# EDAPINENUT/CBGBench

Measured on AMD Instinct MI355X. Metric: denoising graph-steps/s (pocket+ligand graphs x reverse-diffusion steps per second), higher is better.
Workload: dtype f32; 1 GPU; configs/denovo targetdiff sampling, BASELINE configs[1] job: 100 pockets x 10 samples = 1000 graphs per GPU, 3 resident batch(es) of <= 340; N_rec~U[350,650], N_lig~U[10,45], k=32, 9 layers; bench step = 1 reverse-diffusion step of the job at each of 5 time blocks; graphs_per_gpu=1000, nodes_per_gpu=521351, denoising_steps_per_bench_step=5, graph_steps_per_bench_step_per_gpu=5000, ranks_seen=1, launch=stream launches, streams=3, edge_workgroups=256, devices_by_uuid=1

## Files before the change

cbgbench_amd/csrc/api.hip:

```cpp
#include <hip/hip_runtime.h>

#include <cmath>
#include <cstdarg>
#include <cstdio>
#include <cstring>
#include <cstdlib>
#include <vector>

#include "../../include/cbgx.h"
#ifdef CBGX_XCHECK
#include "../../include/cbgx_xcheck.h"
#endif
#include "kernels.h"
#include "layout.h"
#include "workspace.h"

using namespace cbgx;

static thread_local char g_err[512] = "";

namespace cbgx {
int set_error(int code, const char* fmt, ...) {
    va_list ap;
    va_start(ap, fmt);
// ... 328 lines not shown
        HIP_TRY(launch_knn_reg(x, graph_ptr, n_graphs, n_nodes, w.nbr, w.deg, s, w.act.rows, w.act.count));
        HIP_TRY(launch_gate_mfma(packed, x, w.nbr, w.deg, n_nodes, w.e_w, s, w.act.rows, w.act.count));
    }
    NodeList src{nullptr, nullptr};
    if (g_edge_impl != 1) {
        HIP_TRY(launch_mark_seed(gen_flag, gen_flag, n_nodes, w.fa1, s));
        HIP_TRY(launch_mark_nbr(w.act.rows, w.act.count, n_nodes, w.nbr, w.deg, w.fa1, s));
        HIP_TRY(launch_build_active(w.fa1, n_nodes, w.A1.rows, w.A1.count, s));
        src = w.A1;
    }
    const float* xc = x;
    const NodeBufs& b = w.set[0];
    for (int l = 0; l < num_layers; ++l) {
        float* xn = (l == num_layers - 1) ? x_out : w.xbuf[l & 1];
        HIP_TRY(launch_attention(false, packed + GATE_SIZE + (size_t)l * ATT_SIZE, xc, h, w.nbr, w.deg, lig_flag, gen_flag,
                                 w.e_w, n_nodes, b.P, b.Qt, b.q, xn, nullptr, w.act.rows, w.act.count, src.rows, src.count, s));
        xc = xn;
    }
    return CBGX_OK;
}

size_t cbgx_workspace_bytes(int n_nodes, int n_graphs) {
    (void)n_graphs;
    return carve(nullptr, n_nodes).total;
}

int cbgx_knn_graph(const float* x, const int32_t* graph_ptr, int n_graphs, int n_nodes, int k, int32_t* nbr,
                   int32_t* deg, void* stream) {
    if (k != KNN) return fail(CBGX_E_INVALID, "knn_graph: only k=%d is supported (got %d)", KNN, k);
    if (n_nodes < 0 || n_graphs < 0) return fail(CBGX_E_INVALID, "knn_graph: negative size");
    if (n_nodes == 0) return CBGX_OK;
// ... 36 lines not shown
}

int cbgx_h2x_attention(const float* packed, int layer, const float* x, const float* h, const int32_t* nbr,
                       const int32_t* deg, const uint8_t* lig_flag, const uint8_t* gen_flag, const float* e_w,
                       int n_nodes, float* x_out, float* delta_x, void* workspace, size_t workspace_bytes,
                       void* stream) {
    if (n_nodes == 0) return CBGX_OK;
    if (!packed || !x || !h || !nbr || !deg || !lig_flag || !gen_flag || !e_w || !x_out || !workspace || layer < 0 ||
        n_nodes < 0)
        return fail(CBGX_E_INVALID, "h2x_attention: bad argument");
    Workspace w;
    if (int rc = carve_checked("h2x_attention", workspace, workspace_bytes, n_nodes, w)) return rc;
    const NodeBufs& b = w.set[0];
    HIP_TRY(launch_build_active(gen_flag, n_nodes, w.act.rows, w.act.count, (hipStream_t)stream));
    HIP_TRY(launch_attention(false, packed + h2x_off(layer), x, h, nbr, deg, lig_flag, gen_flag, e_w, n_nodes, b.P,
                             b.Qt, b.q, x_out, delta_x, w.act.rows, w.act.count, nullptr, nullptr, (hipStream_t)stream));
    return CBGX_OK;
}

int cbgx_node_stage(const float* packed, int layer, int x2h, const float* h, const uint8_t* lig_flag, int n_nodes,
                    const int32_t* rows, const int32_t* n_rows, int q_direct, float* P, float* q, float* Qt, void* stream) {
    if (n_nodes == 0) return CBGX_OK;
    if (!packed || !h || !lig_flag || !P || !q || !Qt || layer < 0 || n_nodes < 0 || (rows == nullptr) != (n_rows == nullptr))
        return fail(CBGX_E_INVALID, "node_stage: bad argument");
    HIP_TRY(launch_node_mfma(packed + (x2h ? x2h_off(layer) : h2x_off(layer)), h, lig_flag, n_nodes, P, q, Qt, rows, n_rows, nullptr,
                             nullptr, (hipStream_t)stream, true, nullptr, nullptr, q_direct != 0));
    return CBGX_OK;
}

static int classifier_head(const float* packed, int num_layers, int num_classes, const float* h, int n_nodes, float* hidden,
                           float* logits, NodeList rows, hipStream_t s) {
// ... 134 lines not shown
}

static hipError_t edge_x2h(const Forward& f, int l, const NodeBufs& b, const float* xc, const float* hc, float* hn) {
    const LayerPlan& p = f.plan[l];
    return launch_edge_x2h_dual(f.packed + x2h_off(l), xc, hc, b.P, b.Qt, b.q, f.w.nbr, f.w.deg, f.lig_flag, f.gen_flag, f.w.e_w,
                                f.n_nodes, hn, p.pp.rows, p.pp.count, p.gen.rows, p.gen.count, p.full_layer, f.s);
}
static hipError_t node_x2h(const Forward& f, int l, const NodeBufs& b, const float* h_in, hipStream_t on) {
    const LayerPlan& p = f.plan[l];
    return launch_node_mfma(f.packed + x2h_off(l), h_in, f.lig_flag, f.n_nodes, b.P, b.q, b.Qt, p.dst.rows, p.dst.count, p.src.rows,
                            p.src.count, on, true, p.gen.rows, p.gen.count, node_qdirect_enabled());
}
static hipError_t block_h2x(const Forward& f, int l, const NodeBufs& b, const float* xc, const float* hn, float* xn) {
    const Workspace& w = f.w;
    return launch_attention(false, f.packed + h2x_off(l), xc, hn, w.nbr, w.deg, f.lig_flag, f.gen_flag, w.e_w, f.n_nodes, b.P, b.Qt, b.q,
                            xn, nullptr, w.act.rows, w.act.count, w.A1.rows, w.A1.count, f.s);
}

static int forward_fused(const Forward& f) {
    const Workspace& w = f.w;
    hipStream_t s = f.s;
    auto add_x2h = [&](NodeStageJobs& jobs, int l) {
        const LayerPlan& p = f.plan[l];
        const NodeBufs& b = w.set[l & 1];
        add_node_stage_jobs(jobs, f.packed + x2h_off(l), b.P, b.q, b.Qt, p.dst.rows, p.dst.count, p.src.rows, p.src.count, p.fold_flag);
    };
    NodeStageJobs jobs;
    jobs.n = 0;
    add_x2h(jobs, 0);
    HIP_TRY(launch_node_stage_jobs(jobs, f.h, f.lig_flag, f.n_nodes, s));
    const float *xc = f.x, *hc = f.h;
    for (int l = 0; l < f.num_layers; ++l) {
        float *hn, *xn;
        HIP_TRY(begin_layer(f, l, hn, xn));
        HIP_TRY(edge_x2h(f, l, w.set[l & 1], xc, hc, hn));
        jobs.n = 0;
        add_node_stage_jobs(jobs, f.packed + h2x_off(l), w.set[2].P, w.set[2].q, w.set[2].Qt, w.act.rows, w.act.count, w.A1.rows,
                            w.A1.count);
        if (l + 1 < f.num_layers) add_x2h(jobs, l + 1);
        HIP_TRY(launch_node_stage_jobs(jobs, hn, f.lig_flag, f.n_nodes, s));
        HIP_TRY(launch_edge_mfma(false, f.packed + h2x_off(l), xc, hn, w.set[2].P, w.set[2].Qt, w.nbr, w.deg, f.lig_flag, f.gen_flag, w.e_w,
                                 f.n_nodes, xn, nullptr, w.act.rows, w.act.count, s));
        xc = xn;
        hc = hn;
    }
    return CBGX_OK;
}

static int forward_two_streams(const Forward& f, AuxStream* aux) {
    hipStream_t s = f.s;
    HIP_TRY(node_x2h(f, 0, f.w.set[0], f.h, s));
    const float *xc = f.x, *hc = f.h;
    for (int l = 0; l < f.num_layers; ++l) {
        float *hn, *xn;
        HIP_TRY(begin_layer(f, l, hn, xn));
        if (l > 0) HIP_TRY(hipStreamWaitEvent(s, aux->join, 0));
        HIP_TRY(edge_x2h(f, l, f.w.set[l & 1], xc, hc, hn));
// ... 276 lines not shown
```

cbgbench_amd/csrc/dispatch.hip:

```cpp
#include <hip/hip_runtime.h>
#include <stdint.h>

#include "kernels.h"
#include "layout.h"

namespace cbgx {

#ifdef CBGX_XCHECK
int g_edge_impl = 0;
#endif

#define CBGX_LAUNCH_CHECK()                            \
    do {                                               \
        hipError_t _e = hipGetLastError();             \
        if (_e != hipSuccess) return _e;               \
    } while (0)

hipError_t launch_knn(const float* x, const int32_t* graph_ptr, int n_graphs, int n_nodes, int32_t* nbr,
                      int32_t* deg, hipStream_t s) {
    if (n_nodes == 0) return hipSuccess;
#ifdef CBGX_XCHECK
    if (g_edge_impl == 1) return launch_knn_v1(x, graph_ptr, n_graphs, n_nodes, nbr, deg, s);
#endif
    return launch_knn_reg(x, graph_ptr, n_graphs, n_nodes, nbr, deg, s);
}

hipError_t launch_gate(const float* packed, const float* x, const int32_t* nbr, const int32_t* deg, int n_nodes,
                       float* e_w, hipStream_t s) {
    if (n_nodes == 0) return hipSuccess;
#ifdef CBGX_XCHECK
    if (g_edge_impl == 1) return launch_gate_v1(packed, x, nbr, deg, n_nodes, e_w, s);
#endif
    return launch_gate_mfma(packed, x, nbr, deg, n_nodes, e_w, s);
}

hipError_t launch_attention(bool x2h, const float* att, const float* x, const float* h, const int32_t* nbr,
                            const int32_t* deg, const uint8_t* lig, const uint8_t* gen, const float* e_w, int n_nodes,
                            float* P, float* Qt, float* qbuf, float* out, float* dx_out, const int* act, const int* act_count,
                            const int* src, const int* src_count, hipStream_t s) {
    if (n_nodes == 0) return hipSuccess;
#ifdef CBGX_XCHECK
    if (g_edge_impl == 1) return launch_attention_v1(x2h, att, x, h, nbr, deg, lig, gen, e_w, n_nodes, P, Qt, out, dx_out, s);
#endif
    hipError_t e0 = launch_node_mfma(att, h, lig, n_nodes, P, qbuf, Qt, act, act_count, src, src_count, s, x2h);
    if (e0 != hipSuccess) return e0;
    return launch_edge_mfma(x2h, att, x, h, P, Qt, nbr, deg, lig, gen, e_w, n_nodes, out, dx_out, act, act_count, s);
}

__global__ void pack_copy_kernel(const float* __restrict__ src, int src_ld, int src_off, int transpose,
                                 float* __restrict__ dst, int dst_ld, int rows, int cols) {
    int idx = blockIdx.x * blockDim.x + threadIdx.x;
    if (idx >= rows * cols) return;
    int i = idx / cols, j = idx % cols;
    dst[(size_t)i * dst_ld + j] = transpose ? src[(size_t)j * src_ld + i + src_off] : src[(size_t)i * src_ld + j + src_off];
}

__global__ void pack_copy_multi_kernel(PackBatch b) {
    const PackPiece& pc = b.p[blockIdx.y];
    const int total = pc.rows * pc.cols;
    for (int idx = blockIdx.x * blockDim.x + threadIdx.x; idx < total; idx += gridDim.x * blockDim.x) {
// ... 28 lines not shown
```

cbgbench_amd/csrc/edge_body.h:

```cpp
#pragma once
#include <hip/hip_runtime.h>
#include <stdint.h>

#include "edge_common.h"
#include "layout.h"

#ifndef CBGX_EDGE_MIN_WAVES
#define CBGX_EDGE_MIN_WAVES 2
#endif
#ifndef CBGX_EDGE_EARLY_HEADER
#define CBGX_EDGE_EARLY_HEADER 1
#endif
#ifndef CBGX_EDGE_EARLY_LOADS
#define CBGX_EDGE_EARLY_LOADS 1
#endif
#ifndef CBGX_EDGE_WAVE_MAJOR
#define CBGX_EDGE_WAVE_MAJOR 1
#endif

namespace cbgx {

constexpr int EDGE_MIN_WAVES = CBGX_EDGE_MIN_WAVES;
__host__ __device__ __forceinline__ int edge_active_waves(int n_items, int n_wg, int waves) {
    const int per_wg = (n_items + n_wg - 1) / (n_wg > 0 ? n_wg : 1);
// ... 114 lines not shown
        out0 = MFMA(fmaxf(ya.x, 0.f), bb.x, out0);
        out1 = MFMA(fmaxf(ya.y, 0.f), bb.y, out1);
        out0 = MFMA(fmaxf(yb.x, 0.f), bb.z, out0);
        out1 = MFMA(fmaxf(yb.y, 0.f), bb.w, out1);
    }
    return out0 + out1;
}

struct ItemGeom {
    int node, d, lig_i;
    float xi, yi, zi;
    int j0[2];
};
__device__ __forceinline__ int e1_id(int raw, int e, int d, int self) { return e < d ? raw : self; }

template <bool X2H, int WAVES, bool LISTED, bool PP, bool F16 = false>
__device__ __forceinline__ void edge_body(
    float* __restrict__ lds, float* __restrict__ lds_mu, const int wg, const int n_wg,
    const float* __restrict__ att, const float* __restrict__ x, const float* __restrict__ h,
    const float* __restrict__ P, const float* __restrict__ Qt, const int32_t* __restrict__ nbr,
    const int32_t* __restrict__ deg, const uint8_t* __restrict__ lig, const uint8_t* __restrict__ gen,
    const float* __restrict__ e_w, int n_nodes, float* __restrict__ out, float* __restrict__ dx_out,
    const int* __restrict__ act_arg, const int* __restrict__ act_count) {
    const int* __restrict__ act = LISTED ? act_arg : nullptr;
    static_assert(!PP || (X2H && LISTED), "the protein-only kernel is an x2h work-list kernel");
    static_assert(!F16 || X2H, "split-f16 scores and aggregation: x2h only");
    static_assert(PP_IMG_SIZE == IMG_SIZE_X2H, "both x2h images fill the same LDS array");
    constexpr int IMG = X2H ? (int)IMG_SIZE_X2H : (int)IMG_SIZE_H2X;
    auto copy_fixed_nodes = [&]() {
        if (!X2H && act) {
            for (int n = wg * (WAVES * 64) + threadIdx.x; n < n_nodes; n += n_wg * WAVES * 64) {
                unsigned gn = gen[n];
                float px = x[3 * n], py = x[3 * n + 1], pz = x[3 * n + 2];
                asm volatile("" : "+v"(gn), "+v"(px), "+v"(py), "+v"(pz));
                if (!gn) {
                    out[3 * n] = px; out[3 * n + 1] = py; out[3 * n + 2] = pz;
                    if (dx_out) { dx_out[3 * n] = 0.f; dx_out[3 * n + 1] = 0.f; dx_out[3 * n + 2] = 0.f; }
                }
            }
        }
    };
// ... 39 lines not shown
        const unsigned oc = vop(4 * c), oq = vop(16 * q);
        r0 = ldoi(nrow, oc); r1 = ldoi(nrow, oc + 64);
        nb0 = ldoi4(nrow, oq); nb1 = ldoi4(nrow, oq + 64);
    };
    {
        const floatx4* src = reinterpret_cast<const floatx4*>(att + (PP ? A_IMG_PP : A_IMG));
        floatx4* dst = reinterpret_cast<floatx4*>(lds);
        constexpr int NV = (IMG / 4 + WAVES * 64 - 1) / (WAVES * 64);
        if constexpr (WAVES >= 8) {
            floatx4 v[NV];
#pragma unroll
            for (int u = 0; u < NV; ++u) {
                const int t = threadIdx.x + u * (WAVES * 64);
                v[u] = src[t < IMG / 4 ? t : IMG / 4 - 1];
            }
            __builtin_amdgcn_sched_barrier(0);
            if (CBGX_EDGE_EARLY_HEADER && has_item) first_header();
            copy_fixed_nodes();
            __builtin_amdgcn_sched_barrier(0);
#pragma unroll
            for (int u = 0; u < NV; ++u) {
                const int t = threadIdx.x + u * (WAVES * 64);
                if (t < IMG / 4) dst[t] = v[u];
            }
        } else {
            if (CBGX_EDGE_EARLY_HEADER && has_item) first_header();
            copy_fixed_nodes();
            constexpr int NVC = 20;
#pragma unroll 1
            for (int u0 = 0; u0 < NV; u0 += NVC) {
                floatx4 v[NVC];
#pragma unroll
                for (int u = 0; u < NVC; ++u) {
                    const int t = threadIdx.x + (u0 + u) * (WAVES * 64);
                    v[u] = src[t < IMG / 4 ? t : IMG / 4 - 1];
                }
                __builtin_amdgcn_sched_barrier(0);
#pragma unroll
// ... 51 lines not shown
            dist0[hf] = edge_len(g.xi, g.yi, g.zi, ldo1(sbase(x), 12u * j), ldo1(sbase(x), 12u * j + 4), ldo1(sbase(x), 12u * j + 8));
        }
        const gptr pdp = sbase(P + (size_t)i * PROW);
        const unsigned o0 = (unsigned)g.j0[0] * (PROW * 4) + (2 * H + 4 * q) * 4, o1 = (unsigned)g.j0[1] * (PROW * 4) + (2 * H + 4 * q) * 4;
#pragma unroll
        for (int t = 0; t < 8; ++t) { pd[t] = ldo4(pdp, oq + 64 * t); ps0[t] = ldo4(sbase(P), o0 + 64 * t); }
#pragma unroll
        for (int t = 0; t < 8; ++t) ps1[t] = ldo4(sbase(P), o1 + 64 * t);
    }

    for (int k = i_begin; k < i_end; k += i_step) {
        const int i = __builtin_amdgcn_readfirstlane(g.node), d = g.d, lig_i = g.lig_i;
        const bool more = k + i_step < i_end;
        const int k_next = k + i_step;
        float4 q8a = {0.f, 0.f, 0.f, 0.f}, q8b = {0.f, 0.f, 0.f, 0.f};
        if (PP && CBGX_EDGE_EARLY_LOADS) {
            const gptr qp = sbase(Qt + (size_t)i * H);
            const unsigned oq8 = vop(32 * c);
            q8a = ldo4(qp, oq8); q8b = ldo4(qp, oq8 + 16);
        }
        floatx4 acc0[8], acc1[8];
#pragma unroll
        for (int t = 0; t < 8; ++t) {
            const floatx4 pds = f4(pd[t]) * sck.S;
            acc0[t] = f4(ps0[t]) * sck.S + pds; acc1[t] = f4(ps1[t]) * sck.S + pds;
        }
        __builtin_amdgcn_sched_barrier(0);
        ItemGeom ng;
        const int inext = __builtin_amdgcn_readfirstlane(more ? (act ? act[k_next] : k_next) : i);
        ng.node = inext;
        const int nd_raw = deg[inext];
        const int nlig_raw = PP ? 0 : ldob(sbase(lig), vop((unsigned)inext));
        const gptr xrow = sbase(x + 3 * (size_t)inext);
        const unsigned ozero = vop(0u);
        const float nx_raw = ldo1(xrow, ozero), ny_raw = ldo1(xrow, ozero + 4), nz_raw = ldo1(xrow, ozero + 8);
        const gptr nrow = sbase(nbr + (size_t)inext * KNN);
        const unsigned oc = vop(4 * c);
        const int nr0 = ldoi(nrow, oc), nr1 = ldoi(nrow, oc + 64);
        __builtin_amdgcn_sched_barrier(0);
        float4 qrow[8];
        if (PP && !CBGX_EDGE_EARLY_LOADS) {
            const gptr qp = sbase(Qt + (size_t)i * H);
            const unsigned oq8 = vop(32 * c);
            q8a = ldo4(qp, oq8); q8b = ldo4(qp, oq8 + 16);
        }
        if (!PP) {
            const gptr qp = sbase(Qt + (size_t)i * HEADS * H);
            const unsigned oqr = vop((c * H + 4 * q) * 4);
#pragma unroll
            for (int t = 0; t < 8; ++t) qrow[t] = ldo4(qp, oqr + 64 * t);
        }
        float4 sva[2][4], svb[2][4];
        float4 pa = {0.f, 0.f, 0.f, 0.f}, pb = {0.f, 0.f, 0.f, 0.f};
        if (X2H) {
            const int nbv[4] = {nb0.x, nb0.y, nb0.z, nb0.w};
#pragma unroll
            for (int r = 0; r < 4; ++r) {
                const unsigned o = (unsigned)e1_id(nbv[r], 4 * q + r, d, i) * (PROW * 4) + (3 * H + 4 * c) * 4;
                sva[0][r] = ldo4(sbase(P), o);
                svb[0][r] = ldo4(sbase(P), o + 256);
            }
// ... 9 lines not shown
            const float vm = c + 16 * hf < d ? RBF_UP : 0.f;
#pragma unroll
            for (int s = 0; s < 5; ++s) {
                const float u = dist0[hf] - lds_mu[4 * s + q];
                R[hf][s] = fast_exp(-0.5f * (u * u)) * vm;
            }
        }
        const unsigned long long b0 = __ballot(lg0[0]), b1 = __ballot(lg0[1]);
        const unsigned mask_lig = (unsigned)(b0 & 0xffffull) | ((unsigned)(b1 & 0xffffull) << 16);
        const unsigned mask_valid = d >= 32 ? 0xffffffffu : ((1u << d) - 1u);
        const bool has_lig = PP ? false : (mask_lig & mask_valid) != 0;
        const bool has_prot = PP ? true : ((~mask_lig) & mask_valid) != 0 || d == 0;

        floatx4 sc[2];
        float qun = 1.f;
        sc[0] = edge_major_half<true, PP, F16 ? 1 : 0>(acc0, lg0[0], 0, lds_fk, lds_dwt, lds_ln, R[0], has_prot, has_lig, lig_i, lane, q,
                                                       PP ? lds + PP_WFOLD + 4 * lane : nullptr, qrow, sck, q8a, q8b, khk_inv, &qun);
        __builtin_amdgcn_sched_barrier(0);
        int nlj[2];
        float nxj[2][3];
        {
            ng.d = __builtin_amdgcn_readfirstlane(nd_raw);
            ng.lig_i = __builtin_amdgcn_readfirstlane(nlig_raw);
            ng.xi = __uint_as_float(__builtin_amdgcn_readfirstlane(__float_as_uint(nx_raw)));
            ng.yi = __uint_as_float(__builtin_amdgcn_readfirstlane(__float_as_uint(ny_raw)));
            ng.zi = __uint_as_float(__builtin_amdgcn_readfirstlane(__float_as_uint(nz_raw)));
            ng.j0[0] = c < ng.d ? nr0 : inext;
            ng.j0[1] = c + 16 < ng.d ? nr1 : inext;
#pragma unroll
            for (int hf = 0; hf < 2; ++hf) {
                const int j = ng.j0[hf];
                nlj[hf] = PP ? 0 : ldob(sbase(lig), (unsigned)j);
// ... 320 lines not shown
```

cbgbench_amd/csrc/edge_mfma.hip:

```cpp
#include <hip/hip_runtime.h>
#include <stdint.h>

#include <stdlib.h>

#include <atomic>

#include "edge_common.h"
#include "kernels.h"
#include "layout.h"

namespace cbgx {


__constant__ float c_mu[G] = {0.f, 1.f, 1.25f, 1.5f, 1.75f, 2.f, 2.25f, 2.5f, 2.75f, 3.f,
                              3.5f, 4.f, 4.5f, 5.f, 5.5f, 6.f, 7.f, 8.f, 9.f, 10.f};

}

#include "edge_body.h"

namespace cbgx {

template <bool X2H, int WAVES, bool LISTED>
__global__ __launch_bounds__(WAVES * 64) void edge_mfma_kernel(
// ... 108 lines not shown
    const int idx = blockIdx.x * blockDim.x + threadIdx.x;
    if (idx >= H * H) return;
    if (!pb.x2h[blockIdx.y]) {
        if (idx >= HEADS * H) return;
        const int head = idx >> 7, m = idx & 127, t = m >> 4, q = (m >> 2) & 3, r = m & 3;
        pb.att[blockIdx.y][A_IMG + IMG_WBV + ((64 * t + 16 * q + head) << 2) + r] = pb.wv1[blockIdx.y][idx];
        return;
    }
    const int n = idx >> 7, m = idx & 127;
    const int chunk = 16 * (m >> 6) + 4 * ((m >> 4) & 3) + (m & 3), r = (m >> 2) & 3;
    pb.att[blockIdx.y][A_IMG + IMG_WBV + n * H + (((chunk ^ wbv_swizzle((n >> 3) & 15)) << 2) | r)] = pb.wv1[blockIdx.y][idx];
}

__global__ void pack_pp_image_kernel(PackBlocks pb) {
    const int idx = blockIdx.x * blockDim.x + threadIdx.x;
    if (idx >= (int)PP_IMG_SIZE || !pb.x2h[blockIdx.y]) return;
    float* att = pb.att[blockIdx.y];
    const float* img = att + A_IMG;
    float v;
    if (idx < (int)PP_FRAG_V) v = img[IMG_FRAG_K + 3 * 8 * FRAG_BLK + idx];
    else if (idx < (int)PP_LN) v = img[IMG_FRAG_V + 3 * 8 * FRAG_BLK + (idx - PP_FRAG_V)];
    else if (idx < (int)PP_WBV) v = img[IMG_LN + (idx - PP_LN)];
    else if (idx < (int)PP_WFOLD) v = img[IMG_WBV + (idx - PP_WBV)];
    else {
        const int u = idx - (int)PP_WFOLD;
        const int r = u & 3, lane = (u >> 2) & 63, d = (u >> 8) & 7, t = u >> 11;
        const int c = lane & 15, q = lane >> 4;
        v = pb.wk1[blockIdx.y][(size_t)(8 * c + d) * H + 16 * t + 4 * q + r] * 0.35355339059327376220f;
    }
    att[A_IMG_PP + idx] = v;
}
// ... 96 lines not shown
```

cbgbench_amd/csrc/kernels.h:

```cpp
#pragma once
#include <hip/hip_runtime.h>
#include <stdint.h>

namespace cbgx {

struct AuxStream {
    hipStream_t owner = nullptr;
    hipStream_t s = nullptr;
    hipEvent_t fork = nullptr, join = nullptr, done[2] = {nullptr, nullptr};
};
AuxStream* aux_for(hipStream_t caller);
typedef AuxStream AuxLane;

enum KernelClass { K_KNN = 0, K_GATE, K_NODE_GEMM, K_NODE_QUERY, K_EDGE_X2H, K_EDGE_H2X, K_EDGE_X2H_LISTED, K_EDGE_X2H_BWD, K_EDGE_H2X_BWD,
                   K_TRAIN_GEMM, K_EDGE_X2H_BWD_LISTED, K_EDGE_ROWS_REDUCE, K_NUM_CLASSES };
void profile_mark_begin(int cls, hipStream_t s);
void profile_mark_end(hipStream_t s);
bool profile_is_on();

hipError_t launch_knn(const float* x, const int32_t* graph_ptr, int n_graphs, int n_nodes, int32_t* nbr,
                      int32_t* deg, hipStream_t s);
hipError_t launch_gate(const float* packed, const float* x, const int32_t* nbr, const int32_t* deg, int n_nodes,
                       float* e_w, hipStream_t s);
hipError_t launch_node_gemm(const float* A, int lda, const float* Wt, const float* bias, float* C, int ldc, int M,
                            int nout, int act, hipStream_t s, const int* rows = nullptr, const int* n_rows = nullptr);
hipError_t launch_attention(bool x2h, const float* att, const float* x, const float* h, const int32_t* nbr,
                            const int32_t* deg, const uint8_t* lig, const uint8_t* gen, const float* e_w, int n_nodes,
                            float* P, float* Qt, float* qbuf, float* out, float* dx_out, const int* act, const int* act_count,
                            const int* src, const int* src_count, hipStream_t s);
#ifdef CBGX_XCHECK
extern int g_edge_impl;
hipError_t launch_knn_v1(const float* x, const int32_t* graph_ptr, int n_graphs, int n_nodes, int32_t* nbr, int32_t* deg,
                         hipStream_t s);
hipError_t launch_gate_v1(const float* packed, const float* x, const int32_t* nbr, const int32_t* deg, int n_nodes,
                          float* e_w, hipStream_t s);
hipError_t launch_node_gemm_v1(const float* A, int lda, const float* Wt, const float* bias, float* C, int ldc, int M,
                               int nout, int act, hipStream_t s, const int* rows, const int* n_rows);
hipError_t launch_node_query_v1(const float* att, const float* P, float* Qt, int n_nodes, hipStream_t s);
hipError_t launch_attention_v1(bool x2h, const float* att, const float* x, const float* h, const int32_t* nbr,
                               const int32_t* deg, const uint8_t* lig, const uint8_t* gen, const float* e_w, int n_nodes,
                               float* P, float* Qt, float* out, float* dx_out, hipStream_t s);
#else
constexpr int g_edge_impl = 0;
#endif
// ... 30 lines not shown
                            const unsigned* newmask = nullptr);
hipError_t launch_graph_cache_begin(const float* x, const int32_t* graph_ptr, int n_graphs, const uint8_t* lig, const float* r32sq,
                                    int n, uint8_t* dirty, int* list, int* count, const int32_t* s_nbr, const int32_t* s_deg,
                                    const float* s_ew, int32_t* nbr, int32_t* deg, float* ew, const float* h1, const float* h2,
                                    float* out1, float* out2, hipStream_t s);
hipError_t launch_pack_node_tables(const PackBlocks& pb, hipStream_t s);
hipError_t launch_build_active(const uint8_t* flag, int n, int* list, int* count, hipStream_t s, bool counter_zeroed = false);
hipError_t launch_mark_seed(const uint8_t* a, const uint8_t* b, int n, uint8_t* m, hipStream_t s);
hipError_t launch_mark_from_nbr(const uint8_t* flag, const int32_t* nbr, const int32_t* deg, int n, uint8_t* out,
                                hipStream_t s);
hipError_t launch_mark_nbr(const int* list, const int* count, int n_upper, const int32_t* nbr, const int32_t* deg,
                           uint8_t* m, hipStream_t s);
hipError_t launch_node_mfma(const float* att, const float* h, const uint8_t* lig, int n_nodes, float* P, float* qbuf,
                            float* Qt, const int* act, const int* act_count, const int* src, const int* src_count,
                            hipStream_t s, bool large_lists = false, const int* fold = nullptr, const int* fold_count = nullptr,
                            bool q_direct = false);
bool node_qdirect_enabled();
struct NodeStageJob {
    const float* att;
    float *P, *q, *Qt;
    const int *rows, *n_rows;
    unsigned chunk_mask;
    int proj_only;
    const uint8_t* fold_flag;
};
constexpr int NS_JOBS_MAX = 4;
struct NodeStageJobs { NodeStageJob j[NS_JOBS_MAX]; int n; };
constexpr int NODE_STAGE_MAX_ROWS = 8192;
bool add_node_stage_jobs(NodeStageJobs& jobs, const float* att, float* P, float* qbuf, float* Qt, const int* act,
                         const int* act_count, const int* src, const int* src_count, const uint8_t* fold_flag = nullptr);
hipError_t launch_node_stage_jobs(const NodeStageJobs& jobs, const float* h, const uint8_t* lig, int n_nodes, hipStream_t s);
struct GraphFlags {
    const uint8_t *gen, *lig;
    const uint8_t* D1;
    uint8_t *d1, *a1, *a2, *a3, *D2, *S1, *S2;
};
constexpr int LIST_JOBS_MAX = 20;
struct ListJobs {
    const uint8_t* flag[LIST_JOBS_MAX];
    const uint8_t* flag2[LIST_JOBS_MAX];
    int want2[LIST_JOBS_MAX];
    int* list[LIST_JOBS_MAX];
    int* count[LIST_JOBS_MAX];
    int n_jobs;
};
// ... 12 lines not shown
hipError_t launch_graph_lists(const uint8_t* gen, const uint8_t* lig, const uint8_t* d1_in, const int32_t* nbr, const int32_t* deg,
                              const int32_t* graph_ptr, int n_graphs, const GraphListJobs& jobs, bool cached, bool prune,
                              uint8_t* d1_out, hipStream_t s);
hipError_t launch_build_lists(const ListJobs& jobs, int n, hipStream_t s);
hipError_t launch_split_list(const int* list, const int* count, int n, const uint8_t* flag, int* out1, int* cnt1, int* out0,
                             int* cnt0, hipStream_t s, bool counters_zeroed = false);
int set_edge_workgroup_limit(int n);
hipError_t launch_edge_mfma(bool x2h, const float* att, const float* x, const float* h, const float* P,
                            const float* Qt, const int32_t* nbr, const int32_t* deg, const uint8_t* lig,
                            const uint8_t* gen, const float* e_w, int n_nodes, float* out, float* dx_out,
                            const int* act, const int* act_count, hipStream_t s);
hipError_t launch_edge_x2h_dual(const float* att, const float* x, const float* h, const float* P, const float* Qt,
                                const float* qbuf, const int32_t* nbr, const int32_t* deg, const uint8_t* lig,
                                const uint8_t* gen, const float* e_w, int n_nodes, float* out, const int* list_pp,
                                const int* count_pp, const int* list_gen, const int* count_gen, bool full_layer, hipStream_t s);
void launch_edge_x2h_f16_grid(int grid, const float* att, const float* x, const float* h, const float* P, const float* Qt,
                              const float* qbuf, const int32_t* nbr, const int32_t* deg, const uint8_t* lig, const uint8_t* gen,
                              const float* e_w, int n_nodes, float* out, const int* list_pp, const int* count_pp,
                              const int* list_gen, const int* count_gen, bool full_layer, hipStream_t s);
hipError_t launch_step_prologue(const float* x_lig, const float* c_lig, const int32_t* lig_rows, int n_lig, int C,
                                const float* emb_w, const float* emb_b, const float* ind_w, const float* ind_b, float* x,
                                float* h, hipStream_t s, const int32_t* t_ptr = nullptr);
hipError_t launch_step_epilogue(const float* x_den, const float* logits, const int32_t* lig_rows, const float* x_lig,
                                const float* c_lig, const uint8_t* gen_lig, int n_lig, int C, int t,
                                const float* const* tabs, float log_c, const float* eps, const float* u, float* x_next,
                                float* c_next, int32_t* v_next, hipStream_t s, int32_t* t_ptr = nullptr);
hipError_t launch_step_boundary(const float* x_den, const float* logits, const int32_t* lig_rows, const float* x_lig,
                                const float* c_lig, const uint8_t* gen_lig, int n_lig, int C, int t, const float* const* tabs,
                                float log_c, const float* eps, const float* u, float* x_next, float* c_next, const float* emb_w,
                                const float* emb_b, const float* ind_w, const float* ind_b, float* x, float* h, hipStream_t s);
// ... 46 lines not shown
```

cbgbench_amd/csrc/layout.h:

```cpp
#pragma once
#include <cstddef>

namespace cbgx {

constexpr int H = 128;
constexpr int HEADS = 16;
constexpr int DH = 8;
constexpr int G = 20;
constexpr int KNN = 32;
constexpr int NT = 4;
constexpr int GH = 160;
constexpr int KV_IN = 2 * H + NT + NT * G;
constexpr int PROW = 5 * H;

constexpr size_t GATE_W1 = 0;
constexpr size_t GATE_B1 = GATE_W1 + GH * G;
constexpr size_t GATE_LNG = GATE_B1 + GH;
constexpr size_t GATE_LNB = GATE_LNG + GH;
constexpr size_t GATE_W2 = GATE_LNB + GH;
constexpr size_t GATE_B2 = GATE_W2 + GH;
constexpr size_t GATE_IMG = GATE_B2 + 4;
constexpr size_t GATE_IMG_SIZE = (size_t)(GH / 16) * 5 * 64 + 4 * GH;
constexpr size_t GATE_SIZE = GATE_IMG + GATE_IMG_SIZE;

// ... 10 lines not shown
constexpr size_t A_WQ1T = A_LNQ_B + H;
constexpr size_t A_BQ1 = A_WQ1T + (size_t)H * H;
constexpr size_t A_WBK = A_BQ1 + H;
constexpr size_t A_WBV = A_WBK + (size_t)H * H;
constexpr size_t A_BBV = A_WBV + (size_t)H * H;
constexpr size_t FRAG_BLK = 320;
constexpr size_t FRAG = (size_t)NT * 8 * FRAG_BLK;
constexpr size_t A_IMG = A_BBV + H;
constexpr size_t IMG_FRAG_K = 0;
constexpr size_t IMG_FRAG_V = IMG_FRAG_K + FRAG;
constexpr size_t IMG_WT = IMG_FRAG_V + FRAG;
constexpr size_t IMG_LN = IMG_WT + NT * 2 * H;
constexpr size_t IMG_WBV = IMG_LN + 4 * H;
constexpr size_t IMG_SIZE_H2X = IMG_WBV + (size_t)HEADS * H;
constexpr size_t IMG_SIZE_X2H = IMG_WBV + (size_t)H * H;
constexpr size_t A_NPROJ_FRAG = A_IMG + IMG_SIZE_X2H;
constexpr size_t A_WQ1_FRAG = A_NPROJ_FRAG + (size_t)H * PROW;
constexpr size_t A_WBK_FRAG = A_WQ1_FRAG + (size_t)H * H;
constexpr size_t A_WAKC = A_WBK_FRAG + (size_t)H * H;
constexpr size_t A_BAKC = A_WAKC + (size_t)H * KV_IN;
constexpr size_t A_WAVC = A_BAKC + H;
constexpr size_t A_BAVC = A_WAVC + (size_t)H * KV_IN;
constexpr size_t A_BN2 = A_BAVC + H;
constexpr size_t A_WBKT = A_BN2 + 2 * PROW;
constexpr size_t A_WQ1O = A_WBKT + (size_t)H * H;
constexpr size_t A_WRT = A_WQ1O + (size_t)H * H;
constexpr size_t A_WRC = A_WRT + (size_t)NT * 2 * H * 32;
constexpr size_t A_FRAGV_EM = A_WRC + (size_t)NT * G * 2 * H;
constexpr int RBF_EXP = 12;
constexpr int RBF_KW_MIN = -40;
// ... 30 lines not shown
```

cbgbench_amd/csrc/node_mfma.hip:

```cpp
#include <hip/hip_runtime.h>
#include <stdint.h>
#include <stdlib.h>

#include "kernels.h"
#include "layout.h"

namespace cbgx {

typedef float floatx4 __attribute__((ext_vector_type(4)));
#define MFMA(a, b, c) __builtin_amdgcn_mfma_f32_16x16x4f32((a), (b), (c), 0, 0, 0)
typedef _Float16 half8 __attribute__((ext_vector_type(8)));
#define MFMAH32(a, b, c) __builtin_amdgcn_mfma_f32_16x16x32_f16((a), (b), (c), 0, 0, 0)

__device__ __forceinline__ float4 nld4(const float* p) { return *reinterpret_cast<const float4*>(p); }

__device__ __forceinline__ float nxrow_sum(float v) {
    auto r = __builtin_amdgcn_permlane16_swap(__float_as_uint(v), __float_as_uint(v), false, false);
    v = __uint_as_float(r[0]) + __uint_as_float(r[1]);
    r = __builtin_amdgcn_permlane32_swap(__float_as_uint(v), __float_as_uint(v), false, false);
    return __uint_as_float(r[0]) + __uint_as_float(r[1]);
}

__device__ __forceinline__ float nxrow_max(float v) {
    auto r = __builtin_amdgcn_permlane16_swap(__float_as_uint(v), __float_as_uint(v), false, false);
// ... 517 lines not shown
                                                                const uint8_t* __restrict__ lig, int n_nodes) {
    __shared__ __attribute__((aligned(16))) float qh[16][NS_TPITCH];
    __shared__ __attribute__((aligned(16))) float qt[16][NS_TPITCH];
    __shared__ __attribute__((aligned(16))) float cst[4][H];
    const int tid = threadIdx.x, wave = __builtin_amdgcn_readfirstlane(tid >> 6);
    const NodeStageJob& jb = jobs.j[blockIdx.y];
    const float* __restrict__ att = jb.att;
    float* __restrict__ P = jb.P;
    float* __restrict__ qout = jb.q;
    float* __restrict__ Qt = jb.Qt;
    const int* __restrict__ rows = jb.rows;
    const int* __restrict__ n_rows_ptr = jb.n_rows;
    const unsigned chunk_mask = jb.chunk_mask;
    const bool proj_only = jb.proj_only != 0;
    const uint8_t* __restrict__ fold_flag = jb.fold_flag;
    const int n_rows = rows ? *n_rows_ptr : n_nodes;
    const int n_tiles = (n_rows + 15) / 16;
    if ((int)blockIdx.x >= n_tiles) return;
    if (!proj_only) {
#pragma unroll
        for (int u = tid; u < 4 * H; u += NW * 64) {
            const int k = u >> 7, m = u & (H - 1);
            cst[k][m] = att[(k == 0 ? A_LNQ_G : (k == 1 ? A_LNQ_B : (k == 2 ? A_BQ1 : A_WQ1_CINV))) + m];
        }
    }
    for (int tl = blockIdx.x; tl < n_tiles; tl += gridDim.x) {
        const int row0 = tl * 16;
        int lane;
        asm volatile("v_mbcnt_lo_u32_b32 %0, -1, 0\n\tv_mbcnt_hi_u32_b32 %0, -1, %0" : "=v"(lane));
        const int c = lane & 15, q = lane >> 4;
// ... 135 lines not shown
                for (int u = 0; u < 4; ++u) {
                    acc = MFMAH32(zh[u], bl[u], acc);
                    acc = MFMAH32(zl[u], bh[u], acc);
                    acc = MFMAH32(zh[u], bh[u], acc);
                }
#pragma unroll
                for (int r = 0; r < 4; ++r) {
                    const float o = fmaf(acc[r] * zrinv[r], ci, b1);
                    qt[4 * q + r][col] = o;
                    int orw = orow[r];
                    asm volatile("" : "+v"(orw));
                    if (orw >= 0) qout[(size_t)orw * H + col] = o;
                }
            }
        }
        const bool do_fold = __ballot(fm != 0u) != 0ull;
        float4 b00 = {0.f, 0.f, 0.f, 0.f}, b01 = b00, b10 = b00, b11 = b00;
        if (do_fold) {
            const float* fb = att + A_WBK_FRAG + ((size_t)wave * 2 * 64 + lane) * 8;
            b00 = nld4(fb); b01 = nld4(fb + 4); b10 = nld4(fb + 64 * 8); b11 = nld4(fb + 64 * 8 + 4);
        }
        __syncthreads();
        if (do_fold) {
#pragma unroll
            for (int k = 0; k < HEADS / NW; ++k) {
                const int a = wave + k * NW;
                if (k) {
                    const float* fb = att + A_WBK_FRAG + ((size_t)a * 2 * 64 + lane) * 8;
                    b00 = nld4(fb); b01 = nld4(fb + 4); b10 = nld4(fb + 64 * 8); b11 = nld4(fb + 64 * 8 + 4);
                }
                const float2 qv = *reinterpret_cast<const float2*>(&qt[c][8 * a + 2 * q]);
// ... 550 lines not shown
        hipError_t e = hipMemsetAsync(count, 0, sizeof(int), s);
        if (e != hipSuccess) return e;
    }
    if (n == 0) return hipSuccess;
    hipLaunchKernelGGL(build_active_kernel, dim3((n + BA_THREADS - 1) / BA_THREADS), dim3(BA_THREADS), 0, s, flag, n, list, count);
    return hipGetLastError();
}

constexpr unsigned CHUNKS_ALL = 0x3ffu;
constexpr unsigned CHUNKS_PS = 0x0f0u;
constexpr unsigned CHUNKS_OWN = 0x30fu;
constexpr unsigned CHUNKS_QH = 0x300u;


bool add_node_stage_jobs(NodeStageJobs& jobs, const float* att, float* P, float* qbuf, float* Qt, const int* act,
                         const int* act_count, const int* src, const int* src_count, const uint8_t* fold_flag) {
    if (jobs.n + (act ? 2 : 1) > NS_JOBS_MAX) return false;
    jobs.j[jobs.n++] = NodeStageJob{att, P, qbuf, Qt, act, act_count, act ? CHUNKS_OWN : CHUNKS_ALL, 0, fold_flag};
    if (act) jobs.j[jobs.n++] = NodeStageJob{att, P, qbuf, Qt, src, src_count, CHUNKS_PS, 1, nullptr};
    return true;
}

static void launch_node_stage_grid(const NodeStageJobs& jobs, const float* h, const uint8_t* lig, int n_nodes, hipStream_t s) {
    static const int forced = [] { const char* e = getenv("CBGX_NODE_STAGE_WAVES"); return e ? atoi(e) : 0; }();
    const int tiles = (n_nodes + 15) / 16;
    const int nw = (forced == 4 || forced == 8 || forced == 16) ? forced : NODE_STAGE_WAVES;
    const dim3 grid(min(tiles, 1024), jobs.n);
    if (nw == 4) hipLaunchKernelGGL(node_stage_kernel<4>, grid, dim3(256), 0, s, jobs, h, lig, n_nodes);
    else if (nw == 8) hipLaunchKernelGGL(node_stage_kernel<8>, grid, dim3(512), 0, s, jobs, h, lig, n_nodes);
    else hipLaunchKernelGGL(node_stage_kernel<16>, grid, dim3(1024), 0, s, jobs, h, lig, n_nodes);
}

hipError_t launch_node_stage_jobs(const NodeStageJobs& jobs, const float* h, const uint8_t* lig, int n_nodes, hipStream_t s) {
    if (n_nodes == 0 || jobs.n == 0) return hipSuccess;
    if (n_nodes > NODE_STAGE_MAX_ROWS || jobs.n > NS_JOBS_MAX) return hipErrorInvalidValue;
    profile_mark_begin(K_NODE_QUERY, s);
    launch_node_stage_grid(jobs, h, lig, n_nodes, s);
    profile_mark_end(s);
    return hipGetLastError();
}

bool node_qdirect_enabled() {
    static const bool on = [] { const char* e = getenv("CBGX_NODE_QDIRECT"); return !e || atoi(e) != 0; }();
    return on;
}

hipError_t launch_node_mfma(const float* att, const float* h, const uint8_t* lig, int n_nodes, float* P, float* qbuf,
                            float* Qt, const int* act, const int* act_count, const int* src, const int* src_count,
                            hipStream_t s, bool large_lists, const int* fold, const int* fold_count, bool q_direct) {
    if (n_nodes == 0) return hipSuccess;
    const int tiles = (n_nodes + 63) / 64;
    const int grid = min(tiles, 512);
    const bool small = tiles <= 128 || (act != nullptr && !large_lists);
    auto proj_grid = [&](unsigned mask) {
        const int py = (__builtin_popcount(mask) + NP_CPW - 1) / NP_CPW;
        int gx = NP_RESIDENT_WGS / py;
        if (gx >= 8) gx &= ~7;
        return dim3((unsigned)min(tiles, gx), (unsigned)py);
    };
    const bool fused = n_nodes <= NODE_STAGE_MAX_ROWS;
    const bool direct = q_direct && !fused;
    const unsigned chunks_all = direct ? CHUNKS_ALL & ~CHUNKS_QH : CHUNKS_ALL, chunks_own = direct ? CHUNKS_OWN & ~CHUNKS_QH : CHUNKS_OWN;
    profile_mark_begin(K_NODE_GEMM, s);
    const bool two_jobs = fused && act != nullptr;
// ... 9 lines not shown
            else
                hipLaunchKernelGGL(node_proj_kernel<false>, proj_grid(CHUNKS_PS), dim3(256), 0, s, att, h, lig, P, n_nodes,
                                   (const int*)nullptr, (const int*)nullptr, CHUNKS_PS);
        }
        if (!fused)
            hipLaunchKernelGGL(node_proj_kernel<true>, proj_grid(chunks_own), dim3(256), 0, s, att, h, lig, P, n_nodes, act, act_count,
                               chunks_own);
    }
    profile_mark_end(s);
    hipError_t e = hipGetLastError();
    if (e != hipSuccess) return e;
    profile_mark_begin(K_NODE_QUERY, s);
    if (fused) {
        NodeStageJobs jobs;
        jobs.n = 0;
        add_node_stage_jobs(jobs, att, P, qbuf, Qt, act, act_count, src, src_count);
        launch_node_stage_grid(jobs, h, lig, n_nodes, s);
    } else {
        if (direct)
            hipLaunchKernelGGL(node_query_kernel, dim3(min((n_nodes + NQK_ROWS - 1) / NQK_ROWS, NQK_GRID)), dim3(NQK_THREADS), 0, s, att, h,
                               qbuf, n_nodes, act, act_count);
        else
            hipLaunchKernelGGL(node_qmlp_kernel, dim3(grid, small ? 2 : 1), dim3(256), 0, s, att, P, qbuf, n_nodes, act, act_count);
        if (fold)
            hipLaunchKernelGGL(node_qfold_kernel<4>, dim3(grid, 4), dim3(256), 0, s, att, qbuf, Qt, n_nodes, fold, fold_count);
        else if (small)
            hipLaunchKernelGGL(node_qfold_kernel<4>, dim3(grid, 4), dim3(256), 0, s, att, qbuf, Qt, n_nodes, act, act_count);
        else
            hipLaunchKernelGGL(node_qfold_kernel<16>, dim3(grid, 1), dim3(256), 0, s, att, qbuf, Qt, n_nodes, act, act_count);
    }
    profile_mark_end(s);
    return hipGetLastError();
}

}
```

Measured before the change: 31950 graph-steps/s.

## Fold h2x query projection into edge kernel instead of separate node fold pass

Adds an h2x edge kernel variant that loads the H×H fold weight table into LDS and applies the query fold in registers per edge, reading the raw q rows directly. The node stage now skips its separate query-fold step (node_qfold or the in-kernel fold) for h2x layers, and the pack kernel also builds the fold table for h2x layers. The goal is to cut a kernel launch or pass and the writes and reads of the per-head Qt buffer. In exchange the edge kernel uses more LDS, which can lower occupancy, and does the fold work again for each edge block. It is on by default and can be turned off with CBGX_H2X_FOLD=0.

```diff
diff --git a/cbgbench_amd/csrc/api.hip b/cbgbench_amd/csrc/api.hip
--- a/cbgbench_amd/csrc/api.hip
+++ b/cbgbench_amd/csrc/api.hip
@@ -366,7 +366,7 @@
     for (int l = 0; l < num_layers; ++l) {
         float* xn = (l == num_layers - 1) ? x_out : w.xbuf[l & 1];
         HIP_TRY(launch_attention(false, packed + GATE_SIZE + (size_t)l * ATT_SIZE, xc, h, w.nbr, w.deg, lig_flag, gen_flag,
-                                 w.e_w, n_nodes, b.P, b.Qt, b.q, xn, nullptr, w.act.rows, w.act.count, src.rows, src.count, s));
+                                 w.e_w, n_nodes, b.P, b.Qt, b.q, xn, nullptr, w.act.rows, w.act.count, src.rows, src.count, s, true));
         xc = xn;
     }
     return CBGX_OK;
@@ -433,7 +433,7 @@
     const NodeBufs& b = w.set[0];
     HIP_TRY(launch_build_active(gen_flag, n_nodes, w.act.rows, w.act.count, (hipStream_t)stream));
     HIP_TRY(launch_attention(false, packed + h2x_off(layer), x, h, nbr, deg, lig_flag, gen_flag, e_w, n_nodes, b.P,
-                             b.Qt, b.q, x_out, delta_x, w.act.rows, w.act.count, nullptr, nullptr, (hipStream_t)stream));
+                             b.Qt, b.q, x_out, delta_x, w.act.rows, w.act.count, nullptr, nullptr, (hipStream_t)stream, true));
     return CBGX_OK;
 }
 
@@ -598,7 +598,7 @@
 static hipError_t block_h2x(const Forward& f, int l, const NodeBufs& b, const float* xc, const float* hn, float* xn) {
     const Workspace& w = f.w;
     return launch_attention(false, f.packed + h2x_off(l), xc, hn, w.nbr, w.deg, f.lig_flag, f.gen_flag, w.e_w, f.n_nodes, b.P, b.Qt, b.q,
-                            xn, nullptr, w.act.rows, w.act.count, w.A1.rows, w.A1.count, f.s);
+                            xn, nullptr, w.act.rows, w.act.count, w.A1.rows, w.A1.count, f.s, true);
 }
 
 static int forward_fused(const Forward& f) {
@@ -619,12 +619,17 @@
         HIP_TRY(begin_layer(f, l, hn, xn));
         HIP_TRY(edge_x2h(f, l, w.set[l & 1], xc, hc, hn));
         jobs.n = 0;
+        const bool h2x_fold = h2x_fold_enabled();
         add_node_stage_jobs(jobs, f.packed + h2x_off(l), w.set[2].P, w.set[2].q, w.set[2].Qt, w.act.rows, w.act.count, w.A1.rows,
-                            w.A1.count);
+                            w.A1.count, nullptr, h2x_fold);
         if (l + 1 < f.num_layers) add_x2h(jobs, l + 1);
         HIP_TRY(launch_node_stage_jobs(jobs, hn, f.lig_flag, f.n_nodes, s));
-        HIP_TRY(launch_edge_mfma(false, f.packed + h2x_off(l), xc, hn, w.set[2].P, w.set[2].Qt, w.nbr, w.deg, f.lig_flag, f.gen_flag, w.e_w,
-                                 f.n_nodes, xn, nullptr, w.act.rows, w.act.count, s));
+        if (h2x_fold)
+            HIP_TRY(launch_edge_h2x_fold(f.packed + h2x_off(l), xc, hn, w.set[2].P, w.set[2].q, w.nbr, w.deg, f.lig_flag, f.gen_flag, w.e_w,
+                                         f.n_nodes, xn, nullptr, w.act.rows, w.act.count, s));
+        else
+            HIP_TRY(launch_edge_mfma(false, f.packed + h2x_off(l), xc, hn, w.set[2].P, w.set[2].Qt, w.nbr, w.deg, f.lig_flag, f.gen_flag,
+                                     w.e_w, f.n_nodes, xn, nullptr, w.act.rows, w.act.count, s));
         xc = xn;
         hc = hn;
     }
diff --git a/cbgbench_amd/csrc/dispatch.hip b/cbgbench_amd/csrc/dispatch.hip
--- a/cbgbench_amd/csrc/dispatch.hip
+++ b/cbgbench_amd/csrc/dispatch.hip
@@ -37,13 +37,16 @@
 hipError_t launch_attention(bool x2h, const float* att, const float* x, const float* h, const int32_t* nbr,
                             const int32_t* deg, const uint8_t* lig, const uint8_t* gen, const float* e_w, int n_nodes,
                             float* P, float* Qt, float* qbuf, float* out, float* dx_out, const int* act, const int* act_count,
-                            const int* src, const int* src_count, hipStream_t s) {
+                            const int* src, const int* src_count, hipStream_t s, bool inference) {
     if (n_nodes == 0) return hipSuccess;
 #ifdef CBGX_XCHECK
     if (g_edge_impl == 1) return launch_attention_v1(x2h, att, x, h, nbr, deg, lig, gen, e_w, n_nodes, P, Qt, out, dx_out, s);
 #endif
-    hipError_t e0 = launch_node_mfma(att, h, lig, n_nodes, P, qbuf, Qt, act, act_count, src, src_count, s, x2h);
+    const bool h2x_fold = inference && !x2h && act && h2x_fold_enabled();
+    hipError_t e0 = launch_node_mfma(att, h, lig, n_nodes, P, qbuf, Qt, act, act_count, src, src_count, s, x2h, nullptr, nullptr, false,
+                                     h2x_fold);
     if (e0 != hipSuccess) return e0;
+    if (h2x_fold) return launch_edge_h2x_fold(att, x, h, P, qbuf, nbr, deg, lig, gen, e_w, n_nodes, out, dx_out, act, act_count, s);
     return launch_edge_mfma(x2h, att, x, h, P, Qt, nbr, deg, lig, gen, e_w, n_nodes, out, dx_out, act, act_count, s);
 }
 
diff --git a/cbgbench_amd/csrc/edge_body.h b/cbgbench_amd/csrc/edge_body.h
--- a/cbgbench_amd/csrc/edge_body.h
+++ b/cbgbench_amd/csrc/edge_body.h
@@ -152,7 +152,7 @@
 };
 __device__ __forceinline__ int e1_id(int raw, int e, int d, int self) { return e < d ? raw : self; }
 
-template <bool X2H, int WAVES, bool LISTED, bool PP, bool F16 = false>
+template <bool X2H, int WAVES, bool LISTED, bool PP, bool F16 = false, bool HFOLD = false>
 __device__ __forceinline__ void edge_body(
     float* __restrict__ lds, float* __restrict__ lds_mu, const int wg, const int n_wg,
     const float* __restrict__ att, const float* __restrict__ x, const float* __restrict__ h,
@@ -163,6 +163,8 @@
     const int* __restrict__ act = LISTED ? act_arg : nullptr;
     static_assert(!PP || (X2H && LISTED), "the protein-only kernel is an x2h work-list kernel");
     static_assert(!F16 || X2H, "split-f16 scores and aggregation: x2h only");
+    static_assert(!HFOLD || (!X2H && LISTED && WAVES >= 8), "the in-register fold of h2x: the listed 8-wave kernel");
+    constexpr bool QFOLD = PP || HFOLD;
     static_assert(PP_IMG_SIZE == IMG_SIZE_X2H, "both x2h images fill the same LDS array");
     constexpr int IMG = X2H ? (int)IMG_SIZE_X2H : (int)IMG_SIZE_H2X;
     auto copy_fixed_nodes = [&]() {
@@ -232,6 +234,14 @@
                 const int t = threadIdx.x + u * (WAVES * 64);
                 v[u] = src[t < IMG / 4 ? t : IMG / 4 - 1];
             }
+            constexpr int NF = HFOLD ? H * H / 4 / (WAVES * 64) : 1;
+            static_assert(!HFOLD || NF * 4 * WAVES * 64 == H * H, "fold table: NF float4 per thread exactly");
+            floatx4 vf[NF];
+            if constexpr (HFOLD) {
+                const floatx4* srcf = reinterpret_cast<const floatx4*>(att + A_IMG_PP + PP_WFOLD);
+#pragma unroll
+                for (int u = 0; u < NF; ++u) vf[u] = srcf[threadIdx.x + u * (WAVES * 64)];
+            }
             __builtin_amdgcn_sched_barrier(0);
             if (CBGX_EDGE_EARLY_HEADER && has_item) first_header();
             copy_fixed_nodes();
@@ -240,6 +250,11 @@
             for (int u = 0; u < NV; ++u) {
                 const int t = threadIdx.x + u * (WAVES * 64);
                 if (t < IMG / 4) dst[t] = v[u];
+            }
+            if constexpr (HFOLD) {
+                floatx4* dstf = reinterpret_cast<floatx4*>(lds + IMG_H2X_WFOLD);
+#pragma unroll
+                for (int u = 0; u < NF; ++u) dstf[threadIdx.x + u * (WAVES * 64)] = vf[u];
             }
         } else {
             if (CBGX_EDGE_EARLY_HEADER && has_item) first_header();
@@ -321,7 +336,7 @@
         const bool more = k + i_step < i_end;
         const int k_next = k + i_step;
         float4 q8a = {0.f, 0.f, 0.f, 0.f}, q8b = {0.f, 0.f, 0.f, 0.f};
-        if (PP && CBGX_EDGE_EARLY_LOADS) {
+        if (QFOLD && CBGX_EDGE_EARLY_LOADS) {
             const gptr qp = sbase(Qt + (size_t)i * H);
             const unsigned oq8 = vop(32 * c);
             q8a = ldo4(qp, oq8); q8b = ldo4(qp, oq8 + 16);
@@ -346,12 +361,12 @@
         const int nr0 = ldoi(nrow, oc), nr1 = ldoi(nrow, oc + 64);
         __builtin_amdgcn_sched_barrier(0);
         float4 qrow[8];
-        if (PP && !CBGX_EDGE_EARLY_LOADS) {
+        if (QFOLD && !CBGX_EDGE_EARLY_LOADS) {
             const gptr qp = sbase(Qt + (size_t)i * H);
             const unsigned oq8 = vop(32 * c);
             q8a = ldo4(qp, oq8); q8b = ldo4(qp, oq8 + 16);
         }
-        if (!PP) {
+        if (!QFOLD) {
             const gptr qp = sbase(Qt + (size_t)i * HEADS * H);
             const unsigned oqr = vop((c * H + 4 * q) * 4);
 #pragma unroll
@@ -391,8 +406,9 @@
 
         floatx4 sc[2];
         float qun = 1.f;
-        sc[0] = edge_major_half<true, PP, F16 ? 1 : 0>(acc0, lg0[0], 0, lds_fk, lds_dwt, lds_ln, R[0], has_prot, has_lig, lig_i, lane, q,
-                                                       PP ? lds + PP_WFOLD + 4 * lane : nullptr, qrow, sck, q8a, q8b, khk_inv, &qun);
+        const float* lds_wfold = PP ? lds + PP_WFOLD + 4 * lane : (HFOLD ? lds + IMG_H2X_WFOLD + 4 * lane : nullptr);
+        sc[0] = edge_major_half<true, QFOLD, F16 ? 1 : 0>(acc0, lg0[0], 0, lds_fk, lds_dwt, lds_ln, R[0], has_prot, has_lig, lig_i, lane, q,
+                                                          lds_wfold, qrow, sck, q8a, q8b, khk_inv, &qun);
         __builtin_amdgcn_sched_barrier(0);
         int nlj[2];
         float nxj[2][3];
diff --git a/cbgbench_amd/csrc/edge_h2x_fold.hip b/cbgbench_amd/csrc/edge_h2x_fold.hip
--- /dev/null
+++ b/cbgbench_amd/csrc/edge_h2x_fold.hip
@@ -0,0 +1,55 @@
+#include <hip/hip_runtime.h>
+#include <stdint.h>
+#include <stdlib.h>
+
+#include "edge_common.h"
+#include "kernels.h"
+#include "layout.h"
+
+namespace cbgx {
+
+static __constant__ float c_mu[G] = {0.f, 1.f, 1.25f, 1.5f, 1.75f, 2.f, 2.25f, 2.5f, 2.75f, 3.f,
+                                     3.5f, 4.f, 4.5f, 5.f, 5.5f, 6.f, 7.f, 8.f, 9.f, 10.f};
+
+}
+
+#include "edge_body.h"
+
+namespace cbgx {
+
+template <int WAVES>
+__global__ __launch_bounds__(WAVES * 64) void edge_h2x_fold_kernel(
+    const float* __restrict__ att, const float* __restrict__ x, const float* __restrict__ h,
+    const float* __restrict__ P, const float* __restrict__ qbuf, const int32_t* __restrict__ nbr,
+    const int32_t* __restrict__ deg, const uint8_t* __restrict__ lig, const uint8_t* __restrict__ gen,
+    const float* __restrict__ e_w, int n_nodes, float* __restrict__ out, float* __restrict__ dx_out,
+    const int* __restrict__ act, const int* __restrict__ act_count) {
+    __shared__ __attribute__((aligned(16))) float lds[IMG_SIZE_H2X_FOLD];
+    __shared__ float lds_mu[G];
+    edge_body<false, WAVES, true, false, false, true>(lds, lds_mu, blockIdx.x, gridDim.x, att, x, h, P, qbuf, nbr, deg, lig, gen, e_w,
+                                                      n_nodes, out, dx_out, act, act_count);
+}
+
+bool h2x_fold_enabled() {
+    static const bool on = [] { const char* v = getenv("CBGX_H2X_FOLD"); return !(v && v[0] == '0' && v[1] == 0); }();
+    return on;
+}
+
+hipError_t launch_edge_h2x_fold(const float* att, const float* x, const float* h, const float* P, const float* qbuf,
+                                const int32_t* nbr, const int32_t* deg, const uint8_t* lig, const uint8_t* gen, const float* e_w,
+                                int n_nodes, float* out, float* dx_out, const int* act, const int* act_count, hipStream_t s) {
+    if (n_nodes == 0) return hipSuccess;
+    if (!act || !act_count) return hipErrorInvalidValue;
+    if ((size_t)n_nodes * PROW * sizeof(float) >= (1ull << 32)) return hipErrorInvalidValue;
+    constexpr int W = 8;
+    int grid = (n_nodes + EDGE_MIN_WAVES - 1) / EDGE_MIN_WAVES;
+    if (grid > 256) grid = 256;
+    if (grid >= 64) grid &= ~7;
+    profile_mark_begin(K_EDGE_H2X, s);
+    hipLaunchKernelGGL((edge_h2x_fold_kernel<W>), dim3(grid), dim3(W * 64), 0, s, att, x, h, P, qbuf, nbr, deg, lig, gen, e_w, n_nodes,
+                       out, dx_out, act, act_count);
+    profile_mark_end(s);
+    return hipGetLastError();
+}
+
+}
diff --git a/cbgbench_amd/csrc/edge_mfma.hip b/cbgbench_amd/csrc/edge_mfma.hip
--- a/cbgbench_amd/csrc/edge_mfma.hip
+++ b/cbgbench_amd/csrc/edge_mfma.hip
@@ -146,7 +146,8 @@
 
 __global__ void pack_pp_image_kernel(PackBlocks pb) {
     const int idx = blockIdx.x * blockDim.x + threadIdx.x;
-    if (idx >= (int)PP_IMG_SIZE || !pb.x2h[blockIdx.y]) return;
+    if (idx >= (int)PP_IMG_SIZE) return;
+    if (!pb.x2h[blockIdx.y] && idx < (int)PP_WFOLD) return;
     float* att = pb.att[blockIdx.y];
     const float* img = att + A_IMG;
     float v;
diff --git a/cbgbench_amd/csrc/kernels.h b/cbgbench_amd/csrc/kernels.h
--- a/cbgbench_amd/csrc/kernels.h
+++ b/cbgbench_amd/csrc/kernels.h
@@ -27,7 +27,7 @@
 hipError_t launch_attention(bool x2h, const float* att, const float* x, const float* h, const int32_t* nbr,
                             const int32_t* deg, const uint8_t* lig, const uint8_t* gen, const float* e_w, int n_nodes,
                             float* P, float* Qt, float* qbuf, float* out, float* dx_out, const int* act, const int* act_count,
-                            const int* src, const int* src_count, hipStream_t s);
+                            const int* src, const int* src_count, hipStream_t s, bool inference = false);
 #ifdef CBGX_XCHECK
 extern int g_edge_impl;
 hipError_t launch_knn_v1(const float* x, const int32_t* graph_ptr, int n_graphs, int n_nodes, int32_t* nbr, int32_t* deg,
@@ -88,7 +88,7 @@
 hipError_t launch_node_mfma(const float* att, const float* h, const uint8_t* lig, int n_nodes, float* P, float* qbuf,
                             float* Qt, const int* act, const int* act_count, const int* src, const int* src_count,
                             hipStream_t s, bool large_lists = false, const int* fold = nullptr, const int* fold_count = nullptr,
-                            bool q_direct = false);
+                            bool q_direct = false, bool no_fold = false);
 bool node_qdirect_enabled();
 struct NodeStageJob {
     const float* att;
@@ -97,12 +97,14 @@
     unsigned chunk_mask;
     int proj_only;
     const uint8_t* fold_flag;
+    int no_fold;
 };
 constexpr int NS_JOBS_MAX = 4;
 struct NodeStageJobs { NodeStageJob j[NS_JOBS_MAX]; int n; };
 constexpr int NODE_STAGE_MAX_ROWS = 8192;
 bool add_node_stage_jobs(NodeStageJobs& jobs, const float* att, float* P, float* qbuf, float* Qt, const int* act,
-                         const int* act_count, const int* src, const int* src_count, const uint8_t* fold_flag = nullptr);
+                         const int* act_count, const int* src, const int* src_count, const uint8_t* fold_flag = nullptr,
+                         bool no_fold = false);
 hipError_t launch_node_stage_jobs(const NodeStageJobs& jobs, const float* h, const uint8_t* lig, int n_nodes, hipStream_t s);
 struct GraphFlags {
     const uint8_t *gen, *lig;
@@ -145,6 +147,10 @@
                                 const float* qbuf, const int32_t* nbr, const int32_t* deg, const uint8_t* lig,
                                 const uint8_t* gen, const float* e_w, int n_nodes, float* out, const int* list_pp,
                                 const int* count_pp, const int* list_gen, const int* count_gen, bool full_layer, hipStream_t s);
+bool h2x_fold_enabled();
+hipError_t launch_edge_h2x_fold(const float* att, const float* x, const float* h, const float* P, const float* qbuf,
+                                const int32_t* nbr, const int32_t* deg, const uint8_t* lig, const uint8_t* gen, const float* e_w,
+                                int n_nodes, float* out, float* dx_out, const int* act, const int* act_count, hipStream_t s);
 void launch_edge_x2h_f16_grid(int grid, const float* att, const float* x, const float* h, const float* P, const float* Qt,
                               const float* qbuf, const int32_t* nbr, const int32_t* deg, const uint8_t* lig, const uint8_t* gen,
                               const float* e_w, int n_nodes, float* out, const int* list_pp, const int* count_pp,
diff --git a/cbgbench_amd/csrc/layout.h b/cbgbench_amd/csrc/layout.h
--- a/cbgbench_amd/csrc/layout.h
+++ b/cbgbench_amd/csrc/layout.h
@@ -48,6 +48,8 @@
 constexpr size_t IMG_WBV = IMG_LN + 4 * H;
 constexpr size_t IMG_SIZE_H2X = IMG_WBV + (size_t)HEADS * H;
 constexpr size_t IMG_SIZE_X2H = IMG_WBV + (size_t)H * H;
+constexpr size_t IMG_H2X_WFOLD = IMG_SIZE_H2X;
+constexpr size_t IMG_SIZE_H2X_FOLD = IMG_H2X_WFOLD + (size_t)H * H;
 constexpr size_t A_NPROJ_FRAG = A_IMG + IMG_SIZE_X2H;
 constexpr size_t A_WQ1_FRAG = A_NPROJ_FRAG + (size_t)H * PROW;
 constexpr size_t A_WBK_FRAG = A_WQ1_FRAG + (size_t)H * H;
diff --git a/cbgbench_amd/csrc/node_mfma.hip b/cbgbench_amd/csrc/node_mfma.hip
--- a/cbgbench_amd/csrc/node_mfma.hip
+++ b/cbgbench_amd/csrc/node_mfma.hip
@@ -555,6 +555,7 @@
     const unsigned chunk_mask = jb.chunk_mask;
     const bool proj_only = jb.proj_only != 0;
     const uint8_t* __restrict__ fold_flag = jb.fold_flag;
+    const bool no_fold = jb.no_fold != 0;
     const int n_rows = rows ? *n_rows_ptr : n_nodes;
     const int n_tiles = (n_rows + 15) / 16;
     if ((int)blockIdx.x >= n_tiles) return;
@@ -720,7 +721,7 @@
                 }
             }
         }
-        const bool do_fold = __ballot(fm != 0u) != 0ull;
+        const bool do_fold = !no_fold && __ballot(fm != 0u) != 0ull;
         float4 b00 = {0.f, 0.f, 0.f, 0.f}, b01 = b00, b10 = b00, b11 = b00;
         if (do_fold) {
             const float* fb = att + A_WBK_FRAG + ((size_t)wave * 2 * 64 + lane) * 8;
@@ -1301,10 +1302,10 @@
 
 
 bool add_node_stage_jobs(NodeStageJobs& jobs, const float* att, float* P, float* qbuf, float* Qt, const int* act,
-                         const int* act_count, const int* src, const int* src_count, const uint8_t* fold_flag) {
+                         const int* act_count, const int* src, const int* src_count, const uint8_t* fold_flag, bool no_fold) {
     if (jobs.n + (act ? 2 : 1) > NS_JOBS_MAX) return false;
-    jobs.j[jobs.n++] = NodeStageJob{att, P, qbuf, Qt, act, act_count, act ? CHUNKS_OWN : CHUNKS_ALL, 0, fold_flag};
-    if (act) jobs.j[jobs.n++] = NodeStageJob{att, P, qbuf, Qt, src, src_count, CHUNKS_PS, 1, nullptr};
+    jobs.j[jobs.n++] = NodeStageJob{att, P, qbuf, Qt, act, act_count, act ? CHUNKS_OWN : CHUNKS_ALL, 0, fold_flag, no_fold ? 1 : 0};
+    if (act) jobs.j[jobs.n++] = NodeStageJob{att, P, qbuf, Qt, src, src_count, CHUNKS_PS, 1, nullptr, 0};
     return true;
 }
 
@@ -1334,7 +1335,7 @@
 
 hipError_t launch_node_mfma(const float* att, const float* h, const uint8_t* lig, int n_nodes, float* P, float* qbuf,
                             float* Qt, const int* act, const int* act_count, const int* src, const int* src_count,
-                            hipStream_t s, bool large_lists, const int* fold, const int* fold_count, bool q_direct) {
+                            hipStream_t s, bool large_lists, const int* fold, const int* fold_count, bool q_direct, bool no_fold) {
     if (n_nodes == 0) return hipSuccess;
     const int tiles = (n_nodes + 63) / 64;
     const int grid = min(tiles, 512);
@@ -1374,7 +1375,7 @@
     if (fused) {
         NodeStageJobs jobs;
         jobs.n = 0;
-        add_node_stage_jobs(jobs, att, P, qbuf, Qt, act, act_count, src, src_count);
+        add_node_stage_jobs(jobs, att, P, qbuf, Qt, act, act_count, src, src_count, nullptr, no_fold);
         launch_node_stage_grid(jobs, h, lig, n_nodes, s);
     } else {
         if (direct)
@@ -1382,7 +1383,8 @@
                                qbuf, n_nodes, act, act_count);
         else
             hipLaunchKernelGGL(node_qmlp_kernel, dim3(grid, small ? 2 : 1), dim3(256), 0, s, att, P, qbuf, n_nodes, act, act_count);
-        if (fold)
+        if (no_fold) {}
+        else if (fold)
             hipLaunchKernelGGL(node_qfold_kernel<4>, dim3(grid, 4), dim3(256), 0, s, att, qbuf, Qt, n_nodes, fold, fold_count);
         else if (small)
             hipLaunchKernelGGL(node_qfold_kernel<4>, dim3(grid, 4), dim3(256), 0, s, att, qbuf, Qt, n_nodes, act, act_count);
```

After: 32230 graph-steps/s (median of 6 runs). Within noise of the previous version (+0.9%).
